# firechecking/CleanTransformer

Measured on AMD Instinct MI355X. Metric: SFT tokens/sec/step Bloom-560M bf16, higher is better.
Workload: dtype bf16

## Files before the change

### cleantransformer_amd/_lib.py

```python
from __future__ import annotations

import ctypes as C
import os

import torch

from ._build import LIB_PATH as _DEFAULT_LIB_PATH

LIB_PATH = os.environ.get("CTMI_LIB_PATH") or _DEFAULT_LIB_PATH

F32, BF16, F16 = 0, 1, 2
OPT_LEGACY_GRID = 4
OPT_SHADOW_F16 = 2
EPI_NONE, EPI_GELU, EPI_DGELU, EPI_RELU, EPI_DRELU, EPI_GELUG, EPI_MUL = 0, 1, 2, 3, 4, 5, 6
MT_MAX = 24
PROF_CLASSES = ("gemm_fwd", "gemm_dgrad", "gemm_wgrad", "lm_head", "attn_fwd", "attn_bwd", "layernorm", "loss", "optimizer", "reduce", "other")
ABI_VERSION = 16

vp, i64, i32, f32 = C.c_void_p, C.c_int64, C.c_int, C.c_float


class CtmiError(RuntimeError):
    pass


class AttnDesc(C.Structure):
    _fields_ = [(n, i64) for n in ("B", "nh", "Sq", "Sk", "hd",
                                   "q_bs", "q_hs", "q_rs", "k_bs", "k_hs", "k_rs",
                                   "v_bs", "v_hs", "v_rs", "o_bs", "o_hs", "o_rs",
                                   "am_b", "am_h", "am_q", "am_k")] + [("scale", f32), ("causal", i32), ("future_fill", f32), ("dropout_seed", C.c_uint32), ("dropout_p", f32), ("reserved_", i32)]


# ... 17 lines not shown


class BloomBlockGrads(C.Structure):
    _fields_ = [("dout", vp), ("dx", vp)] + [("d" + n, vp) for n in BLK_PARAMS] + \
               [("ws", vp), ("ws_bytes", i64), ("splitk_ws", vp), ("splitk_ws_bytes", i64), ("side_stream", vp),
                ("side_splitk_ws", vp), ("side_splitk_ws_bytes", i64), ("defer_join", i32)]


PROTOTYPES = {
    "ctmi_abi_version": (i32, []),
    "ctmi_last_error": (C.c_char_p, []),
    "ctmi_layernorm_fwd": (i32, [vp, vp, vp, vp, vp, vp, i64, i64, f32, i32, vp]),
    "ctmi_layernorm_bwd_ws": (i64, [i64, i64]),
    "ctmi_layernorm_bwd": (i32, [vp, vp, vp, vp, vp, vp, vp, vp, vp, i32, vp, i64, i64, i32, vp]),
    "ctmi_gemm": (i32, [vp, i64, i32, vp, i64, i32, vp, i64, i64, i64, i64, f32, i32, vp, vp, i32, vp, vp, i32, i32, vp, i64, vp]),
    "ctmi_set_launch_policy": (i32, [i32, i32]),
    "ctmi_get_launch_policy": (i32, [C.POINTER(i32), C.POINTER(i32)]),
    "ctmi_colsum": (i32, [vp, i64, vp, i32, vp, i64, i64, i32, vp]),
    "ctmi_colsum_ws": (i64, [i64, i64]),
    "ctmi_attn_fwd": (i32, [vp, vp, vp, vp, vp, vp, vp, vp, vp, vp, vp, C.POINTER(AttnDesc), i32, vp]),
    "ctmi_attn_bwd": (i32, [vp, vp, vp, vp, vp, vp, vp, vp, vp, vp, vp, vp, vp, vp, vp, vp, C.POINTER(AttnDesc), i32, vp]),
    "ctmi_attn_set_path": (i32, [i32]),
    "ctmi_mask_prep": (i32, [vp, vp, vp, vp, i64, i64, vp]),
    "ctmi_embed_fwd": (i32, [vp, vp, vp, i64, i64, i64, i32, vp, vp]),
    "ctmi_embed_bwd": (i32, [vp, vp, vp, i64, i64, i64, i32, f32, vp]),
    "ctmi_ce_fwd": (i32, [vp, i64, vp, vp, vp, vp, i64, i64, i64, i64, i64, i32, i64, i32, vp]),
    "ctmi_ce_bwd": (i32, [vp, i64, vp, vp, vp, vp, vp, i64, i64, i64, i64, i64, i64, i32, vp]),
    "ctmi_ce_fwd_bwd": (i32, [vp, i64, vp, vp, vp, vp, vp, i64, i64, i64, i64, i64, i64, i32, i64, f32, vp, i32, vp]),
    "ctmi_scale_if": (i32, [vp, i64, i64, i64, vp, f32, vp, i32, vp]),
    "ctmi_scale_if_passes": (i64, []),
# ... 13 lines not shown
    "ctmi_ddp_all_gather": (C.c_int, [C.c_void_p, C.c_void_p, C.c_void_p, C.c_int64, C.c_void_p]),
    "ctmi_ddp_broadcast": (C.c_int, [C.c_void_p, C.c_void_p, C.c_int64, C.c_int, C.c_void_p]),
    "ctmi_ddp_wait": (C.c_int, [C.c_void_p, C.c_void_p]),
    "ctmi_dropout_hash": (C.c_uint32, [C.c_uint32]),
    "ctmi_dropout_keep_hash": (C.c_uint32, [C.c_uint32, C.c_uint32]),
    "ctmi_dropout_threshold": (C.c_uint32, [f32]),
    "ctmi_dropout": (i32, [vp, vp, vp, i64, f32, C.c_uint32, i32, vp]),
    "ctmi_adamw_step": (i32, [C.POINTER(vp), C.POINTER(vp), C.POINTER(vp), C.POINTER(vp), C.POINTER(vp), C.POINTER(i64),
                              i32, f32, f32, f32, f32, f32, i32, i32, i32, f32, vp]),
    "ctmi_adamw_set_hyper": (i32, [vp, f32, f32, f32, f32, f32, i32, i32, i32, f32, vp]),
    "ctmi_adamw_step_dev": (i32, [C.POINTER(vp), C.POINTER(vp), C.POINTER(vp), C.POINTER(vp), C.POINTER(vp), C.POINTER(i64), i32, vp, vp]),
    "ctmi_sgd_step": (i32, [C.POINTER(vp), C.POINTER(vp), C.POINTER(vp), C.POINTER(vp), C.POINTER(i64),
                            i32, f32, f32, f32, f32, i32, vp]),
    "ctmi_cast": (i32, [vp, i32, vp, i32, i64, vp]),
    "ctmi_transpose_cast": (i32, [vp, vp, i32, i64, i64, vp]),
    "ctmi_sumsq": (i32, [vp, i64, vp, i32, vp]),
    "ctmi_scale": (i32, [vp, i64, f32, vp, vp]),
    "ctmi_scale_copy": (i32, [vp, vp, i64, f32, vp]),
    "ctmi_amp_unscale": (i32, [C.POINTER(vp), C.POINTER(i64), i32, vp, vp]),
    "ctmi_amp_update": (i32, [vp, f32, f32, i32, vp]),
    "ctmi_argmax": (i32, [vp, i64, vp, i64, i64, i32, vp]),
    "ctmi_row_lse": (i32, [vp, i64, vp, i64, i64, i32, vp]),
    "ctmi_group_topk": (i32, [vp, i64, vp, vp, f32, vp, vp, i64, i32, i64, i32, i32, vp]),
    "ctmi_scores_filter": (i32, [vp, i64, f32, vp, i64, f32, vp, i64, i64, i64, vp]),
    "ctmi_lora_project": (i32, [vp, i64, vp, i64, i32, vp, i64, i64, i64, i64, f32, i32, vp]),
    "ctmi_lora_expand_add": (i32, [vp, i64, vp, i64, i32, vp, i64, i64, i64, i64, i32, vp]),
    "ctmi_lora_wgrad_ws": (i64, [i64, i64, i64]),
    "ctmi_lora_wgrad": (i32, [vp, i64, vp, i64, vp, i64, i64, i64, i64, f32, vp, i64, i32, vp]),
    "ctmi_probe": (i32, [i32, vp, vp, vp]),
    "ctmi_clock_probe": (i32, [i32, vp, vp]),
# ... 42 lines not shown
```

### cleantransformer_amd/csrc/elementwise.hip

```cpp
#include "common.h"
#include "reduce_jobs.h"
#include "prof.h"
#include <hip/amd_detail/amd_hip_unsafe_atomics.h>

#ifndef CTMI_LN_BWD_PREFETCH
#define CTMI_LN_BWD_PREFETCH 1
#endif

static thread_local char g_err[512] = "";
void ctmi_set_error(const char* fmt, ...) {
    va_list ap; va_start(ap, fmt); vsnprintf(g_err, sizeof(g_err), fmt, ap); va_end(ap);
}
extern "C" const char* ctmi_last_error(void) { return g_err; }
static thread_local bool g_attr_err = false;
void ctmi_dyn_lds(const void* kern, size_t lds_bytes) {
    const hipError_t e = hipFuncSetAttribute(kern, hipFuncAttributeMaxDynamicSharedMemorySize, (int)lds_bytes);
    if (e != hipSuccess) {
        (void)hipGetLastError();
        ctmi_set_error("hipFuncSetAttribute(MaxDynamicSharedMemorySize = %zu bytes) refused: %s", lds_bytes, hipGetErrorString(e));
        g_attr_err = true;
    }
}
bool ctmi_take_attr_error() { const bool r = g_attr_err; g_attr_err = false; return r; }
extern "C" int ctmi_abi_version(void) { return CTMI_ABI_VERSION; }
// ... 1551 lines not shown
        if (c < C && r < R) dst[c * R + r] = Cvt<TD>::from_f(tile[tx][i]);
    }
}
extern "C" int ctmi_transpose_cast(const float* src, void* dst, int dst_dtype, int64_t rows, int64_t cols, void* stream) {
    ProfScope prof__(CTMI_PROF_OTHER, as_stream(stream));
    CTMI_REQUIRE(src && dst && rows > 0 && cols > 0, "transpose_cast: bad args");
    const dim3 grid((unsigned)cdiv64(cols, 64), (unsigned)cdiv64(rows, 64));
    if (dst_dtype == CTMI_F32) hipLaunchKernelGGL((transpose_cast_k<float>), grid, dim3(256), 0, as_stream(stream), src, (float*)dst, rows, cols);
    else if (dst_dtype == CTMI_BF16) hipLaunchKernelGGL((transpose_cast_k<bf16_t>), grid, dim3(256), 0, as_stream(stream), src, (bf16_t*)dst, rows, cols);
    else if (dst_dtype == CTMI_F16) hipLaunchKernelGGL((transpose_cast_k<f16_t>), grid, dim3(256), 0, as_stream(stream), src, (f16_t*)dst, rows, cols);
    else { ctmi_set_error("transpose_cast: unsupported dtype %d", dst_dtype); return CTMI_ERR_UNSUPPORTED; }
    CTMI_CHECK_LAUNCH("transpose_cast");
    return CTMI_OK;
}

__global__ __launch_bounds__(256) void sumsq_k(const float* __restrict__ x, int64_t n, double* __restrict__ out) {
    double s = 0.0;
    for (int64_t i = (int64_t)blockIdx.x * 256 + threadIdx.x; i < n; i += (int64_t)gridDim.x * 256) { const double v = x[i]; s += v * v; }
    for (int o = 32; o > 0; o >>= 1) s += __shfl_xor(s, o, 64);
    __shared__ double sm[4];
    if ((threadIdx.x & 63) == 0) sm[threadIdx.x >> 6] = s;
    __syncthreads();
    if (threadIdx.x == 0) atomicAdd(out, sm[0] + sm[1] + sm[2] + sm[3]);
}
extern "C" int ctmi_sumsq(const float* x, int64_t n, double* out, int accumulate, void* stream) {
    ProfScope prof__(CTMI_PROF_OTHER, as_stream(stream));
    CTMI_REQUIRE(x && out && n >= 0, "sumsq: bad args");
    hipStream_t st = as_stream(stream);
    if (!accumulate) { if (hipMemsetAsync(out, 0, sizeof(double), st) != hipSuccess) { ctmi_set_error("sumsq: memset failed"); return CTMI_ERR_LAUNCH; } }
    if (n == 0) return CTMI_OK;
// ... 203 lines not shown
```

### cleantransformer_amd/csrc/gemm.hip

```cpp
#include "common.h"
#include "reduce_jobs.h"
#include <type_traits>
#include "mma.h"
#include "prof.h"
#include <atomic>
#ifndef CTMI_GEMM_PART
#define CTMI_GEMM_PART (-1)
#endif
#ifndef CTMI_GELU_AUX_WT
#define CTMI_GELU_AUX_WT 0
#endif
#ifndef CTMI_SIDE_PRE8
#define CTMI_SIDE_PRE8 1
#endif
#define CTMI_GEMM_HAS(p) (CTMI_GEMM_PART == -1 || CTMI_GEMM_PART == (p))

constexpr bool glds_k2(bool pp, int wm) { return pp && wm == 4; }
constexpr int glds_ring(bool pp, int wm, bool xlane = false) { return !pp ? 3 : (glds_k2(pp, wm) ? 6 : 4); }
constexpr int glds_patch_bytes(bool pp, int wm, bool xlane = false) { return (pp && !xlane && wm != 4) ? 4 * 8192 : 0; }


template <typename T> struct Tile;
template <> struct Tile<bf16_t> { static constexpr int BM = 128, BN = 128, BK = 64, PADK = 8, PADR = 8; };
template <> struct Tile<f16_t>  { static constexpr int BM = 128, BN = 128, BK = 64, PADK = 8, PADR = 8; };
// ... 103 lines not shown
    return tile[(r16 + (lane & 15)) * PITCH + kofs];
}
template <> __device__ __forceinline__ float OpTile<float, true, 128>::frag(const float* __restrict__ tile, int r16, int lane, int kofs) {
    return tile[kofs * PITCH + r16 + (lane & 15)];
}

struct GemmArgs {
    const void* A; const void* B; void* C;
    int64_t lda, ldb, ldc, M, N, K;
    float alpha; int beta;
    const float* bias; const void* residual; const void* aux_in; void* aux_out;
    int tiles_m, tiles_n, vec_c, vec8;
    int nt_c;
    int splits; int64_t k_per_split; float* slabs;
    int splitk_ok; float* ws; int64_t ws_bytes;
};

constexpr int WG_MAXP = 4;
struct GroupProb { const void* A; const void* B; float* C; float* cs; float* part; float* cspart; int64_t lda, ldb, ldc, M, N, csn; };
struct GroupedArgs : GemmArgs { GroupProb p[WG_MAXP]; const int4* items; int nitems; };
constexpr int WG_PART = 16, WG_COLSUM = 32, WG_HALF1 = 64, WG_COLSUMB = 128;
template <bool GRP, int WM, bool BSUM = false> struct GrpRegs { };
template <int WM> struct GrpRegs<true, WM, false> { f32x4 accs; bool cs_on; };
template <int WM> struct GrpRegs<true, WM, true> { f32x4 accs; bool cs_on; f32x4 accb[4]; bool csb_on; };
#define WG_ONES8 (std::is_same<T, f16_t>::value ? short8{0x3C00, 0x3C00, 0x3C00, 0x3C00, 0x3C00, 0x3C00, 0x3C00, 0x3C00} \
                                                : short8{0x3F80, 0x3F80, 0x3F80, 0x3F80, 0x3F80, 0x3F80, 0x3F80, 0x3F80})

typedef uint32_t u32x4 __attribute__((ext_vector_type(4)));
template <typename TO> __device__ __forceinline__ void store4(TO* p, const float* v);
template <> __device__ __forceinline__ void store4<float>(float* p, const float* v) { *reinterpret_cast<float4*>(p) = make_float4(v[0], v[1], v[2], v[3]); }
// ... 226 lines not shown

template <typename TO, bool AK, bool BKM, int EPI, int WM, int WGN, bool PP, bool RES, bool XLANE, bool GRP, typename GA, typename TE = bf16_t, bool BSUM = false>
__device__ __forceinline__ void glds_body(const GA g) {
    using T = TE;
    static_assert(!GRP || (PP && WM == 4 && WGN == 4 && AK && BKM && EPI == CTMI_EPI_NONE && sizeof(TO) == 4), "grouped launches: weight gradients on the 128x256 ping-pong tile");
    constexpr int NW = 2 * WGN;
    constexpr int BM = WM * 32, BN = WGN * 64, BK = 32, NST = glds_ring(PP, WM, XLANE);
    using TA = GTile<AK, BM>;
    using TB = GTile<BKM, BN>;
    constexpr int STAGE = TA::BYTES + TB::BYTES;
    constexpr int AOFF = 0, BOFF = NST * TA::BYTES;
    constexpr int PA = TA::NINSTR / NW, PB = TB::NINSTR / NW;
    constexpr int LOADS = PA + PB;
    static_assert(PP ? (LOADS == 3 || LOADS == 4) : (LOADS == 4 || LOADS == 6), "vmcnt immediates below assume these DMA piece counts");
    constexpr bool K2 = glds_k2(PP, WM);
    constexpr int FILL = K2 ? NST - 2 : NST - 1;
    constexpr int LAND = K2 ? 2 : 1;
    extern __shared__ __attribute__((aligned(16))) unsigned char smem_raw[];

    const int tiles_m = (int)((g.M + BM - 1) / BM);
    const int tiles_n = (int)((g.N + BN - 1) / BN);
    const int ntile = tiles_m * tiles_n;
    int nwork_;
    if constexpr (GRP) nwork_ = g.nitems; else nwork_ = ntile * g.splits;
    const int nwork = nwork_;
    const int bid = blockIdx.x, G = gridDim.x;
    constexpr int GM = (WM == 8) ? ((AK && BKM) ? 1 : 4) : 8;
    auto decode = [&](int w, int64_t& m0, int64_t& n0, int& split) {
        const int xcd = w & 7, q = nwork >> 3, r8 = nwork & 7;
        const int vid_all = (xcd < r8 ? xcd * (q + 1) : r8 * (q + 1) + (xcd - r8) * q) + (w >> 3);
// ... 114 lines not shown
                float* d = Cl + (int64_t)arow(i) * ldc + 32 * jp;
                st_wt16(d, f32x4{a0, a1, a2, a3});
                st_wt16(d + 4, f32x4{b0, b1, b2, b3});
            }
        if (gs.cs_on) {
            if ((lane >> 4) == 0) {
                float* d = (part ? P.cspart + (half1 ? P.csn : 0) : P.cs) + mw + arow(0) + lane;
                *d = gs.accs[0];
            }
        }
        if constexpr (BSUM) {
            if (gs.csb_on && (lane & 15) == 0) {
                float* d = (part ? P.cspart + (half1 ? P.csn : 0) : P.cs) + nw + (lane >> 4) * 4;
#pragma unroll
                for (int j = 0; j < 4; ++j) *reinterpret_cast<f32x4*>(d + j * 16) = gs.accb[j];
            }
        }
        return;
    }
    if (g.splits > 1) {
        float* S = g.slabs + (int64_t)split * g.M * g.N;
#pragma unroll
        for (int i = 0; i < WM; ++i) {
            const int64_t m = m0 + wr * (WM * 16) + i * 16 + (lane & 15);
            if (m >= g.M) continue;
#pragma unroll
            for (int j = 0; j < 4; ++j) {
                const int64_t n = n0 + wc * 64 + j * 16 + (lane >> 4) * 4;
                if (n >= g.N) continue;
                float v[4] = {acc[i][j][0], acc[i][j][1], acc[i][j][2], acc[i][j][3]};
// ... 401 lines not shown
                    const unsigned char* bs = smem_raw + BOFF + rd * TB::BYTES;
                    short8 af[WM], bf[4];
#pragma unroll
                    for (int j = 0; j < 4; ++j) bf[j] = TB::frag(bs, wc * 64 + j * 16, lane);
#pragma unroll
                    for (int i = 0; i < WM; ++i) af[i] = TA::frag(as, wr * (WM * 16) + arow(i), lane);
                    issue_stage(wrb);
                    wait_stages(FILL - LAND);
                    asm volatile("s_waitcnt lgkmcnt(0)" ::: "memory");
                    __builtin_amdgcn_sched_barrier(0);
                    __builtin_amdgcn_s_barrier();
                    __builtin_amdgcn_sched_barrier(0);
#pragma unroll
                    for (int i = 0; i < WM; ++i)
#pragma unroll
                        for (int j = 0; j < 4; ++j) acc[i][j] = Mma<T>::mma(bf[j], af[i], acc[i][j]);
                    if constexpr (GRP) {
                        if (gs.cs_on) gs.accs = Mma<T>::mma(WG_ONES8, af[0], gs.accs);
                        if constexpr (BSUM) {
                            if (gs.csb_on) {
#pragma unroll
                                for (int j = 0; j < 4; ++j) gs.accb[j] = Mma<T>::mma(bf[j], WG_ONES8, gs.accb[j]);
                            }
                        }
                    }
                    __builtin_amdgcn_sched_barrier(0);
                    __builtin_amdgcn_s_barrier();
                    __builtin_amdgcn_sched_barrier(0);
                    if constexpr ((NST & (NST - 1)) == 0) { rd = (rd + 1) & (NST - 1); wrb = (wrb + 1) & (NST - 1); }
                    else { rd = rd == NST - 1 ? 0 : rd + 1; wrb = wrb == NST - 1 ? 0 : wrb + 1; }
                }
// ... 11 lines not shown
            for (int j = 0; j < 4; ++j) bf[j] = TB::frag(bs, wc * 64 + j * 16, lane);
#pragma unroll
            for (int i = 0; i < WM; ++i) af[i] = TA::frag(as, wr * (WM * 16) + arow(i), lane);
            if (more) {
                issue_stage(wrb);
                stage_issued(); ++inflight; wrb = wrb == NST - 1 ? 0 : wrb + 1;
            }
            wait_stages(inflight - 1 - LAND);
            asm volatile("s_waitcnt lgkmcnt(0)" ::: "memory");
            __builtin_amdgcn_sched_barrier(0);
            __builtin_amdgcn_s_barrier();
            __builtin_amdgcn_sched_barrier(0);
#pragma unroll
            for (int i = 0; i < WM; ++i)
#pragma unroll
                for (int j = 0; j < 4; ++j) acc[i][j] = Mma<T>::mma(bf[j], af[i], acc[i][j]);
            if constexpr (GRP) {
                if (gs.cs_on) gs.accs = Mma<T>::mma(WG_ONES8, af[0], gs.accs);
                if constexpr (BSUM) {
                    if (gs.csb_on) {
#pragma unroll
                        for (int j = 0; j < 4; ++j) gs.accb[j] = Mma<T>::mma(bf[j], WG_ONES8, gs.accb[j]);
                    }
                }
            }
            __builtin_amdgcn_sched_barrier(0);
            __builtin_amdgcn_s_barrier();
            __builtin_amdgcn_sched_barrier(0);
            rd = rd == NST - 1 ? 0 : rd + 1;
            --inflight;
            if (++tc < ntc) continue;
// ... 315 lines not shown
    if (g.splits > 1) {
        const int64_t total = g.M * g.N;
        const unsigned rg = (unsigned)std::min<int64_t>(cdiv64(total, 256), 4096);
        hipLaunchKernelGGL((splitk_reduce<TO>), dim3(rg), dim3(256), 0, st, g.slabs, reinterpret_cast<TO*>(g.C), g.ldc, g.M, g.N, g.splits, g.alpha, g.beta);
        CTMI_CHECK_LAUNCH("gemm_splitk_reduce");
    }
    return CTMI_OK;
}

int ctmi_gemm_bf16_nt(GemmArgs& g, int epi, bool fast, hipStream_t st);
int ctmi_gemm_bf16_nn(GemmArgs& g, int epi, bool fast, hipStream_t st);
int ctmi_gemm_bf16_tn(GemmArgs& g, int epi, bool fast, hipStream_t st);
int ctmi_gemm_f16_nt(GemmArgs& g, int epi, bool fast, hipStream_t st);
int ctmi_gemm_f16_nn(GemmArgs& g, int epi, bool fast, hipStream_t st);
int ctmi_gemm_f16_tn(GemmArgs& g, int epi, bool fast, hipStream_t st);
static int gemm_unsupported(int ak, int bk, int epi, int out_f32) {
    ctmi_set_error("gemm: unsupported combination a_kmajor=%d b_kmajor=%d epilogue=%d out_f32=%d", ak, bk, epi, out_f32);
    return CTMI_ERR_UNSUPPORTED;
}

#if CTMI_GEMM_HAS(1)
int ctmi_gemm_bf16_nt(GemmArgs& g, int epi, bool fast, hipStream_t st) {
    if (epi == CTMI_EPI_NONE) return gemm_launch<bf16_t, bf16_t, false, false, CTMI_EPI_NONE>(g, fast, st);
    if (epi == CTMI_EPI_GELU) return gemm_launch<bf16_t, bf16_t, false, false, CTMI_EPI_GELU>(g, fast, st);
    if (epi == CTMI_EPI_GELUG) return gemm_launch<bf16_t, bf16_t, false, false, CTMI_EPI_GELUG>(g, fast, st);
    if (epi == CTMI_EPI_RELU) return gemm_launch<bf16_t, bf16_t, false, false, CTMI_EPI_RELU>(g, fast, st);
    if (epi == CTMI_EPI_DGELU) return gemm_launch<bf16_t, bf16_t, false, false, CTMI_EPI_DGELU>(g, fast, st);
    return gemm_unsupported(0, 0, epi, 0);
}
#endif
#if CTMI_GEMM_HAS(2)
int ctmi_gemm_bf16_nn(GemmArgs& g, int epi, bool fast, hipStream_t st) {
    if (epi == CTMI_EPI_NONE) return gemm_launch<bf16_t, bf16_t, false, true, CTMI_EPI_NONE>(g, fast, st);
    if (epi == CTMI_EPI_DGELU) return gemm_launch<bf16_t, bf16_t, false, true, CTMI_EPI_DGELU>(g, fast, st);
    if (epi == CTMI_EPI_MUL) return gemm_launch<bf16_t, bf16_t, false, true, CTMI_EPI_MUL>(g, fast, st);
    if (epi == CTMI_EPI_DRELU) return gemm_launch<bf16_t, bf16_t, false, true, CTMI_EPI_DRELU>(g, fast, st);
    if (epi == CTMI_EPI_GELU) return gemm_launch<bf16_t, bf16_t, false, true, CTMI_EPI_GELU>(g, fast, st);
    return gemm_unsupported(0, 1, epi, 0);
}
#endif
#if CTMI_GEMM_HAS(3)
int ctmi_gemm_bf16_tn(GemmArgs& g, int epi, bool fast, hipStream_t st) {
    if (epi == CTMI_EPI_NONE) return gemm_launch<bf16_t, float, true, true, CTMI_EPI_NONE>(g, fast, st);
    return gemm_unsupported(1, 1, epi, 1);
}

#include <map>
#include <mutex>
#include <vector>
namespace {
struct WgShape { int64_t M[WG_MAXP], N[WG_MAXP]; int cs[WG_MAXP]; int n; int64_t ksteps; int slots; int split;
    bool operator<(const WgShape& o) const {
        if (n != o.n) return n < o.n;
        if (ksteps != o.ksteps) return ksteps < o.ksteps;
        if (slots != o.slots) return slots < o.slots;
        if (split != o.split) return split < o.split;
        for (int i = 0; i < n; ++i) { if (M[i] != o.M[i]) return M[i] < o.M[i]; if (N[i] != o.N[i]) return N[i] < o.N[i]; if (cs[i] != o.cs[i]) return cs[i] < o.cs[i]; }
        return false;
    }
};
// ... 192 lines not shown
int ctmi_gemm_f16_nn(GemmArgs& g, int epi, bool fast, hipStream_t st) {
    using T = f16_t;
    if (epi == CTMI_EPI_NONE) return gemm_launch<T, T, false, true, CTMI_EPI_NONE>(g, fast, st);
    if (epi == CTMI_EPI_DGELU) return gemm_launch<T, T, false, true, CTMI_EPI_DGELU>(g, fast, st);
    if (epi == CTMI_EPI_MUL) return gemm_launch<T, T, false, true, CTMI_EPI_MUL>(g, fast, st);
    if (epi == CTMI_EPI_DRELU) return gemm_launch<T, T, false, true, CTMI_EPI_DRELU>(g, fast, st);
    if (epi == CTMI_EPI_GELU) return gemm_launch<T, T, false, true, CTMI_EPI_GELU>(g, fast, st);
    return gemm_unsupported(0, 1, epi, 0);
}
#endif
#if CTMI_GEMM_HAS(6)
int ctmi_gemm_f16_tn(GemmArgs& g, int epi, bool fast, hipStream_t st) {
    if (epi == CTMI_EPI_NONE) return gemm_launch<f16_t, float, true, true, CTMI_EPI_NONE>(g, fast, st);
    return gemm_unsupported(1, 1, epi, 1);
}
#endif

#if CTMI_GEMM_HAS(0)
static int gemm_dispatch_bf16(GemmArgs& g, int ak, int bk, int epi, int out_f32, bool fast, hipStream_t st) {
    if (!ak && !bk && !out_f32) return ctmi_gemm_bf16_nt(g, epi, fast, st);
    if (!ak && bk && !out_f32) return ctmi_gemm_bf16_nn(g, epi, fast, st);
    if (ak && bk && out_f32) return ctmi_gemm_bf16_tn(g, epi, fast, st);
    return gemm_unsupported(ak, bk, epi, out_f32);
}

static int gemm_dispatch_f16(GemmArgs& g, int ak, int bk, int epi, int out_f32, bool fast, hipStream_t st) {
    if (!ak && !bk && !out_f32) return ctmi_gemm_f16_nt(g, epi, fast, st);
    if (!ak && bk && !out_f32) return ctmi_gemm_f16_nn(g, epi, fast, st);
    if (ak && bk && out_f32) return ctmi_gemm_f16_tn(g, epi, fast, st);
    return gemm_unsupported(ak, bk, epi, out_f32);
}

static int gemm_dispatch_f32(GemmArgs& g, int ak, int bk, int epi, bool fast, hipStream_t st) {
    using T = float;
    if (!ak && !bk) {
        if (epi == CTMI_EPI_NONE) return gemm_launch<T, float, false, false, CTMI_EPI_NONE>(g, fast, st);
        if (epi == CTMI_EPI_GELU) return gemm_launch<T, float, false, false, CTMI_EPI_GELU>(g, fast, st);
        if (epi == CTMI_EPI_GELUG) return gemm_launch<T, float, false, false, CTMI_EPI_GELUG>(g, fast, st);
        if (epi == CTMI_EPI_RELU) return gemm_launch<T, float, false, false, CTMI_EPI_RELU>(g, fast, st);
        if (epi == CTMI_EPI_DGELU) return gemm_launch<T, float, false, false, CTMI_EPI_DGELU>(g, fast, st);
    }
    if (!ak && bk) {
        if (epi == CTMI_EPI_NONE) return gemm_launch<T, float, false, true, CTMI_EPI_NONE>(g, fast, st);
        if (epi == CTMI_EPI_DGELU) return gemm_launch<T, float, false, true, CTMI_EPI_DGELU>(g, fast, st);
        if (epi == CTMI_EPI_MUL) return gemm_launch<T, float, false, true, CTMI_EPI_MUL>(g, fast, st);
        if (epi == CTMI_EPI_DRELU) return gemm_launch<T, float, false, true, CTMI_EPI_DRELU>(g, fast, st);
        if (epi == CTMI_EPI_GELU) return gemm_launch<T, float, false, true, CTMI_EPI_GELU>(g, fast, st);
    }
    if (ak && bk && epi == CTMI_EPI_NONE) return gemm_launch<T, float, true, true, CTMI_EPI_NONE>(g, fast, st);
    return gemm_unsupported(ak, bk, epi, 1);
}

extern "C" int ctmi_gemm(const void* A, int64_t lda, int a_kmajor, const void* B, int64_t ldb, int b_kmajor,
                         void* C, int64_t ldc, int64_t M, int64_t N, int64_t K,
                         float alpha, int beta, const float* bias, const void* residual, int epilogue,
                         const void* aux_in, void* aux_out, int out_f32, int dtype,
                         void* workspace, int64_t workspace_bytes, void* stream) {
    CTMI_REQUIRE(A && B && C, "gemm: null operand");
    CTMI_REQUIRE(M > 0 && N > 0 && K > 0, "gemm: bad shape M=%lld N=%lld K=%lld", (long long)M, (long long)N, (long long)K);
    CTMI_REQUIRE(lda >= (a_kmajor ? M : K) && ldb >= (b_kmajor ? N : K) && ldc >= N, "gemm: leading dimension too small");
    CTMI_REQUIRE((epilogue != CTMI_EPI_GELU && epilogue != CTMI_EPI_GELUG) || aux_out, "gemm: GELU epilogues need aux_out");
    CTMI_REQUIRE((epilogue != CTMI_EPI_DGELU && epilogue != CTMI_EPI_DRELU && epilogue != CTMI_EPI_MUL) || aux_in, "gemm: dGELU/dReLU/MUL epilogues need aux_in");
    CTMI_REQUIRE(dtype == CTMI_F32 || dtype == CTMI_BF16 || dtype == CTMI_F16, "gemm: unsupported dtype %d", dtype);
    ProfScope prof__((M >= 65536 || N >= 65536 || K >= 65536) ? CTMI_PROF_LM_HEAD
                     : (a_kmajor && b_kmajor ? CTMI_PROF_GEMM_WGRAD : ((!a_kmajor && b_kmajor) ? CTMI_PROF_GEMM_DGRAD : CTMI_PROF_GEMM_FWD)), as_stream(stream));
    const int es = dtype == CTMI_F32 ? 4 : 2;
    const int vec = 16 / es;
    const int bkt = dtype == CTMI_F32 ? Tile<float>::BK : Tile<bf16_t>::BK;
    GemmArgs g;
    g.A = A; g.B = B; g.C = C; g.lda = lda; g.ldb = ldb; g.ldc = ldc; g.M = M; g.N = N; g.K = K;
    g.alpha = alpha; g.beta = beta; g.bias = bias; g.residual = residual; g.aux_in = aux_in; g.aux_out = aux_out;
    g.tiles_m = (int)cdiv64(M, 128); g.tiles_n = (int)cdiv64(N, 128);
    const int64_t ntile = (int64_t)g.tiles_m * g.tiles_n;
    CTMI_REQUIRE(ntile < (1LL << 27), "gemm: too many tiles");
    const bool vec_a = (lda % vec == 0) && ((((uintptr_t)A) & 15) == 0) && ((a_kmajor ? M : K) % vec == 0);
    const bool vec_b = (ldb % vec == 0) && ((((uintptr_t)B) & 15) == 0) && ((b_kmajor ? N : K) % vec == 0);
    const bool fast = vec_a && vec_b;
    auto al = [](const void* p, int bytes) { return p == nullptr || ((((uintptr_t)p) & (bytes - 1)) == 0); };
    const int cbytes = (out_f32 || dtype == CTMI_F32) ? 16 : 8;
    g.vec_c = (ldc % 4 == 0) && al(C, cbytes) && al(residual, 4 * es) && al(aux_in, 4 * es) && al(aux_out, 4 * es) && al(bias, 16);
    static int nt_on = -1;
    if (nt_on < 0) { const char* e = getenv("CTMI_GEMM_NT"); nt_on = e ? atoi(e) : 1; }
    g.nt_c = nt_on && (M * N * (int64_t)((out_f32 || dtype == CTMI_F32) ? 4 : 2) > (1LL << 30)) ? 1 : 0;
    g.vec8 = g.vec_c && (ldc % 8 == 0) && al(C, 16) && al(residual, 16) && al(aux_in, 16) && al(aux_out, 16);
    g.splits = 1; g.k_per_split = K; g.slabs = nullptr;
    g.splitk_ok = (workspace != nullptr && epilogue == CTMI_EPI_NONE && bias == nullptr && residual == nullptr) ? 1 : 0;
    g.ws = reinterpret_cast<float*>(workspace); g.ws_bytes = workspace_bytes;
    if (workspace != nullptr && epilogue == CTMI_EPI_NONE && bias == nullptr && residual == nullptr && ntile < 384 && K >= 8 * bkt) {
        int64_t want = std::min<int64_t>(8, cdiv64(512, ntile));
        want = std::min<int64_t>(want, K / (4 * bkt));
        want = std::min<int64_t>(want, workspace_bytes / (int64_t)(M * N * sizeof(float)));
        if (want > 1) {
            const int64_t kps = cdiv64(cdiv64(K, want), bkt) * bkt;
            g.splits = (int)cdiv64(K, kps); g.k_per_split = kps; g.slabs = reinterpret_cast<float*>(workspace);
            if (g.splits <= 1) { g.splits = 1; g.k_per_split = K; g.slabs = nullptr; }
        }
    }
    if (dtype == CTMI_F32) return gemm_dispatch_f32(g, a_kmajor, b_kmajor, epilogue, fast, as_stream(stream));
    if (dtype == CTMI_F16) return gemm_dispatch_f16(g, a_kmajor, b_kmajor, epilogue, out_f32, fast, as_stream(stream));
    return gemm_dispatch_bf16(g, a_kmajor, b_kmajor, epilogue, out_f32, fast, as_stream(stream));
}
#endif

#if CTMI_GEMM_PART == 9
#ifndef CTMI_ONE_KERNEL
#define CTMI_ONE_KERNEL bf16_t, false, true, 0, 4, 4, true, false, false
#endif
template __global__ void gemm_glds_kernel<CTMI_ONE_KERNEL>(GemmArgs);
#endif
```

### cleantransformer_amd/models/modeling_bloom.py

```python
from __future__ import annotations

import math
import os as _os
from typing import Optional

import torch

from .. import _lib, ops, rng
from ..generation.generation_util import GenerationMixin
from ..transformer import LayerNorm

Tensor = torch.Tensor


class BloomConfig():

    def __init__(
            self,
            vocab_size=250880,
            hidden_size=64,
            n_layer=2,
            num_attention_heads=8,
            layer_norm_epsilon=1e-5,
            initializer_range=0.02,
# ... 297 lines not shown
        h2, weight = ctx.saved_tensors
        B, S, H = ctx.shape
        V = weight.shape[0]
        d2 = dlogits.reshape(B * S, V)
        wc = ops.compute_weight(weight, h2.dtype)
        tie = ctx.tie
        tied = tie is not None and tie.embed_wants
        sync = getattr(weight, "_ct_tied_sync", None) if tied else None
        pre = sync.prescale(weight) if sync is not None else None
        Vp = ops.ZERO_PADDED.pop(d2.data_ptr(), (None, None))[0] if d2.is_cuda else None
        want_dw = ctx.needs_input_grad[1]
        wpad = getattr(weight, "_ct_shadow_pad", None)
        if Vp is not None and d2.stride() == (Vp, 1) and wpad is not None and wpad.shape[0] == Vp and wpad.dtype == h2.dtype:
            dp = d2.as_strided((B * S, Vp), (Vp, 1))
            dh = ops.linear_dgrad(dp, wpad)
            dw = ops.linear_wgrad(dp, h2, alpha=1.0 if pre is None else pre)[:V] if want_dw else None
        else:
            d2 = ops._c(d2)
            rows = sync.chunk_rows(V, H) if pre is not None else V
            if rows < V:
                dw = torch.empty((V, H), dtype=torch.float32, device=d2.device)
                sync.announce(tie.n_tokens, d2.device)
                for c0 in range(0, V, rows):
                    c1 = min(V, c0 + rows)
                    ops.gemm(d2[:, c0:], V, True, h2, H, True, c1 - c0, H, B * S, out=dw[c0:c1], out_f32=True, alpha=pre)
                    sync.begin(dw[c0:c1])
                tie.pending, tie.early = dw, sync
                dh = ops.linear_dgrad(d2, wc)
                return dh.view(B, S, H), None, None
            dh = ops.linear_dgrad(d2, wc)
            dw = ops.linear_wgrad(d2, h2, alpha=1.0 if pre is None else pre) if want_dw else None
        if tied:
            tie.pending = dw
            if pre is not None:
                sync.announce(tie.n_tokens, dw.device)
                sync.begin(dw)
                tie.early = sync
            dw = None
        return dh.view(B, S, H), dw, None


_FUSED_CE = _os.environ.get("CTMI_FUSED_CE", "1") != "0"


class ShiftedCrossEntropyFn(torch.autograd.Function):

# ... 209 lines not shown
```

### cleantransformer_amd/ops.py

```python
from __future__ import annotations

import contextlib
import os
import ctypes as C
import math
import threading
from typing import Optional, Tuple

import torch

from . import _lib
from ._lib import AttnDesc, BF16, F16, F32, check

Tensor = torch.Tensor


def _p(t: Optional[Tensor]):
    return None if t is None else C.c_void_p(t.data_ptr())


def _stream():
    return C.c_void_p(torch.cuda.current_stream().cuda_stream)


# ... 143 lines not shown
def linear_fwd(x2d: Tensor, w: Tensor, bias: Optional[Tensor] = None, residual: Optional[Tensor] = None,
               epilogue: int = _lib.EPI_NONE, aux_out: Optional[Tensor] = None, tag: Optional[str] = None,
               out: Optional[Tensor] = None) -> Tensor:
    T, K = x2d.shape
    N = w.shape[0]
    return gemm(x2d, K, False, w, K, False, T, N, K, bias=bias, residual=residual, epilogue=epilogue, aux_out=aux_out, tag=tag, out=out)


def linear_dgrad(dy: Tensor, w: Tensor, epilogue: int = _lib.EPI_NONE, aux_in: Optional[Tensor] = None,
                 residual: Optional[Tensor] = None) -> Tensor:
    T, Nout = dy.shape
    Kin = w.shape[1]
    return gemm(dy, Nout, False, w, Kin, True, T, Kin, Nout, epilogue=epilogue, aux_in=aux_in, residual=residual)


def linear_wgrad(dy: Tensor, x2d: Tensor, out: Optional[Tensor] = None, accumulate: bool = False, alpha: float = 1.0) -> Tensor:
    T, Nout = dy.shape
    Kin = x2d.shape[1]
    return gemm(dy, Nout, True, x2d, Kin, True, Nout, Kin, T, out=out, out_f32=True, beta=int(accumulate), alpha=alpha)


def wgrad_grouped(problems, in_out: bool = False):
    lib = _lib.load()
    arr = (_lib.WgradProblem * len(problems))()
    outs = []
    T = problems[0][0].shape[0]
    for i, (dy, x, want_db) in enumerate(problems):
        _need_cuda(dy, x)
        assert dy.is_contiguous() and x.is_contiguous() and dy.shape[0] == T and x.shape[0] == T
        n_out, n_in = dy.shape[1], x.shape[1]
        dw = torch.empty((n_in, n_out) if in_out else (n_out, n_in), dtype=torch.float32, device=dy.device)
        db = torch.empty(n_out, dtype=torch.float32, device=dy.device) if want_db else None
        arr[i].dy, arr[i].x, arr[i].dw, arr[i].db = dy.data_ptr(), x.data_ptr(), dw.data_ptr(), (None if db is None else db.data_ptr())
        arr[i].n_out, arr[i].n_in, arr[i].in_out = n_out, n_in, int(in_out)
# ... 871 lines not shown
```

### include/ctmi355.h

```cpp
#ifndef CTMI355_H
#define CTMI355_H

#include <stdint.h>

#ifdef __cplusplus
extern "C" {
#endif

#define CTMI_ABI_VERSION 16

enum ctmi_dtype { CTMI_F32 = 0, CTMI_BF16 = 1, CTMI_F16 = 2 };
enum ctmi_status { CTMI_OK = 0, CTMI_ERR_ARG = -1, CTMI_ERR_LAUNCH = -2, CTMI_ERR_UNSUPPORTED = -3 };

int ctmi_abi_version(void);
const char* ctmi_last_error(void);

int ctmi_layernorm_fwd(const void* x, const float* w, const float* b, void* y, float* mean, float* rstd,
                       int64_t rows, int64_t cols, float eps, int dtype, void* stream);
int64_t ctmi_layernorm_bwd_ws(int64_t rows, int64_t cols);
int ctmi_layernorm_bwd(const void* dy, const void* x, const float* w, const float* mean, const float* rstd,
                       const void* dres, void* dx, float* dw, float* db, int accumulate, float* ws,
                       int64_t rows, int64_t cols, int dtype, void* stream);

enum ctmi_epilogue { CTMI_EPI_NONE = 0, CTMI_EPI_GELU = 1, CTMI_EPI_DGELU = 2, CTMI_EPI_RELU = 3, CTMI_EPI_DRELU = 4,
                     CTMI_EPI_GELUG = 5, CTMI_EPI_MUL = 6 };
int ctmi_gemm(const void* A, int64_t lda, int a_kmajor, const void* B, int64_t ldb, int b_kmajor,
              void* C, int64_t ldc, int64_t M, int64_t N, int64_t K,
              float alpha, int beta, const float* bias, const void* residual, int epilogue,
              const void* aux_in, void* aux_out, int out_f32, int dtype,
              void* workspace, int64_t workspace_bytes, void* stream);

typedef struct ctmi_wgrad_problem {
    const void* dy; const void* x;
    float* dw; float* db;
    int64_t n_out, n_in;
    int in_out; int pad_;
} ctmi_wgrad_problem;
int ctmi_wgrad_grouped(const ctmi_wgrad_problem* problems , int count, int64_t T, int dtype,
                       void* workspace , int64_t workspace_bytes, void* stream);

int ctmi_set_launch_policy(int shared, int reserve_cus);
int ctmi_get_launch_policy(int* shared , int* reserve_cus );

enum ctmi_prof_class {
    CTMI_PROF_GEMM_FWD = 0,
// ... 84 lines not shown
                    int decoupled, int mutate_grad, float grad_scale, void* stream);
int ctmi_adamw_set_hyper(void* hyper_dev , float lr, float beta1, float beta2, float eps, float weight_decay,
                         int step, int decoupled, int mutate_grad, float grad_scale, void* stream);
int ctmi_adamw_step_dev(float* const* p , float* const* g , float* const* m , float* const* v ,
                        void* const* shadow , const int64_t* n , int count,
                        const void* hyper_dev , void* stream);
int ctmi_sgd_step(float* const* p, float* const* g, float* const* buf ,
                  void* const* shadow, const int64_t* n, int count, float lr, float momentum, float dampening,
                  float weight_decay, int first_step, void* stream);

int ctmi_amp_unscale(float* const* g , const int64_t* n , int count, float* state , void* stream);
int ctmi_amp_update(float* state , float growth, float backoff, int interval, void* stream);

int ctmi_cast(const void* src, int src_dtype, void* dst, int dst_dtype, int64_t n, void* stream);
int ctmi_transpose_cast(const float* src, void* dst, int dst_dtype, int64_t rows, int64_t cols, void* stream);
int ctmi_sumsq(const float* x, int64_t n, double* out, int accumulate, void* stream);
int ctmi_scale(float* x, int64_t n, float s, const float* s_dev , void* stream);
int ctmi_scale_copy(const float* src, float* dst, int64_t n, float s, void* stream);
int ctmi_argmax(const void* x, int64_t ld, int64_t* out, int64_t rows, int64_t cols, int dtype, void* stream);

int ctmi_row_lse(const void* x, int64_t ld, float* stats , int64_t rows, int64_t cols, int dtype, void* stream);
int ctmi_group_topk(const void* x, int64_t ld, const float* stats, const float* add, float add_mul, float* out_val ,
                    int64_t* out_idx , int64_t groups, int group, int64_t cols, int k, int dtype, void* stream);
int ctmi_scores_filter(const float* x, int64_t ld, float divisor, const float* thr, int64_t thr_stride, float fill, float* out,
                       int64_t ldo, int64_t rows, int64_t cols, void* stream);

#define CTMI_REDUCE_MAX_JOBS 16
typedef struct ctmi_reduce_job {
    const float* src; float* dst; int64_t n; int64_t part_stride; int32_t nparts; int32_t accumulate; float alpha; int32_t pad_;
} ctmi_reduce_job;
// ... 55 lines not shown
```

Measured before the change: 230,800.

## Compute LM-head weight gradient via transposed activations and transposed-output NN GEMM

Adds a 16-bit tiled transpose kernel and a new GEMM variant that computes the LM-head weight gradient in NN form over pre-transposed hidden states, storing the fp32 result transposed by swapping MMA operands. The old path used the TN (both k-major) wgrad kernel for the large vocab x hidden product. The intent is to use the faster NN ping-pong tile path for this large GEMM, paying for it with one extra transpose of the hidden activations and an extra buffer. A fallback to the original GEMM remains when shapes or alignment do not qualify.

Result: no change. 231,500 (median of 6 runs) (+0.3%).

```diff
diff --git a/cleantransformer_amd/_lib.py b/cleantransformer_amd/_lib.py
--- a/cleantransformer_amd/_lib.py
+++ b/cleantransformer_amd/_lib.py
@@ -15,7 +15,7 @@
 EPI_NONE, EPI_GELU, EPI_DGELU, EPI_RELU, EPI_DRELU, EPI_GELUG, EPI_MUL = 0, 1, 2, 3, 4, 5, 6
 MT_MAX = 24
 PROF_CLASSES = ("gemm_fwd", "gemm_dgrad", "gemm_wgrad", "lm_head", "attn_fwd", "attn_bwd", "layernorm", "loss", "optimizer", "reduce", "other")
-ABI_VERSION = 16
+ABI_VERSION = 17
 
 vp, i64, i32, f32 = C.c_void_p, C.c_int64, C.c_int, C.c_float
 
@@ -63,6 +63,7 @@
     "ctmi_layernorm_bwd_ws": (i64, [i64, i64]),
     "ctmi_layernorm_bwd": (i32, [vp, vp, vp, vp, vp, vp, vp, vp, vp, i32, vp, i64, i64, i32, vp]),
     "ctmi_gemm": (i32, [vp, i64, i32, vp, i64, i32, vp, i64, i64, i64, i64, f32, i32, vp, vp, i32, vp, vp, i32, i32, vp, i64, vp]),
+    "ctmi_lmhead_wgrad": (i32, [vp, i64, vp, i64, vp, i64, i64, i64, i64, f32, i32, vp]),
     "ctmi_set_launch_policy": (i32, [i32, i32]),
     "ctmi_get_launch_policy": (i32, [C.POINTER(i32), C.POINTER(i32)]),
     "ctmi_colsum": (i32, [vp, i64, vp, i32, vp, i64, i64, i32, vp]),
@@ -106,6 +107,7 @@
                             i32, f32, f32, f32, f32, i32, vp]),
     "ctmi_cast": (i32, [vp, i32, vp, i32, i64, vp]),
     "ctmi_transpose_cast": (i32, [vp, vp, i32, i64, i64, vp]),
+    "ctmi_transpose16": (i32, [vp, i64, vp, i64, i64, i64, vp]),
     "ctmi_sumsq": (i32, [vp, i64, vp, i32, vp]),
     "ctmi_scale": (i32, [vp, i64, f32, vp, vp]),
     "ctmi_scale_copy": (i32, [vp, vp, i64, f32, vp]),
diff --git a/cleantransformer_amd/csrc/elementwise.hip b/cleantransformer_amd/csrc/elementwise.hip
--- a/cleantransformer_amd/csrc/elementwise.hip
+++ b/cleantransformer_amd/csrc/elementwise.hip
@@ -1589,6 +1589,48 @@
     return CTMI_OK;
 }
 
+__global__ __launch_bounds__(256) void transpose16_k(const uint16_t* __restrict__ src, int64_t ld_src, uint16_t* __restrict__ dst, int64_t ld_dst,
+                                                     int64_t R, int64_t C) {
+    __shared__ uint32_t tile[64 * 33];
+    const int t = threadIdx.x;
+    const int64_t r0 = (int64_t)blockIdx.y * 64, c0 = (int64_t)blockIdx.x * 64;
+#pragma unroll
+    for (int i = 0; i < 2; ++i) {
+        const int id = t + 256 * i, row = id >> 3, cc = id & 7;
+        const int64_t r = r0 + row, c = c0 + cc * 8;
+        if (r < R && c < C) {
+            const uint4 v = *reinterpret_cast<const uint4*>(src + r * ld_src + c);
+            uint32_t* d = tile + row * 33 + cc * 4;
+            d[0] = v.x; d[1] = v.y; d[2] = v.z; d[3] = v.w;
+        }
+    }
+    __syncthreads();
+    const int rc = t & 7, cp = t >> 3;
+    const int64_t r = r0 + rc * 8, c = c0 + cp * 2;
+    if (r < R && c < C) {
+        uint32_t w[8];
+#pragma unroll
+        for (int k = 0; k < 8; ++k) w[k] = tile[(rc * 8 + k) * 33 + cp];
+        uint4 lo, hi;
+        lo.x = (w[0] & 0xffffu) | (w[1] << 16); lo.y = (w[2] & 0xffffu) | (w[3] << 16); lo.z = (w[4] & 0xffffu) | (w[5] << 16); lo.w = (w[6] & 0xffffu) | (w[7] << 16);
+        hi.x = (w[0] >> 16) | (w[1] & 0xffff0000u); hi.y = (w[2] >> 16) | (w[3] & 0xffff0000u); hi.z = (w[4] >> 16) | (w[5] & 0xffff0000u); hi.w = (w[6] >> 16) | (w[7] & 0xffff0000u);
+        *reinterpret_cast<uint4*>(dst + c * ld_dst + r) = lo;
+        *reinterpret_cast<uint4*>(dst + (c + 1) * ld_dst + r) = hi;
+    }
+}
+extern "C" int ctmi_transpose16(const void* src, int64_t ld_src, void* dst, int64_t ld_dst, int64_t rows, int64_t cols, void* stream) {
+    ProfScope prof__(CTMI_PROF_OTHER, as_stream(stream));
+    CTMI_REQUIRE(src && dst && rows > 0 && cols > 0 && ld_src >= cols && ld_dst >= rows, "transpose16: bad args");
+    if ((rows | cols | ld_src | ld_dst) % 8 != 0 || !aligned16(src) || !aligned16(dst) || cdiv64(rows, 64) > 65535) {
+        ctmi_set_error("transpose16: rows, cols and both row pitches must be multiples of 8 and the pointers 16-byte aligned (rows <= 4193280)");
+        return CTMI_ERR_UNSUPPORTED;
+    }
+    const dim3 grid((unsigned)cdiv64(cols, 64), (unsigned)cdiv64(rows, 64));
+    hipLaunchKernelGGL(transpose16_k, grid, dim3(256), 0, as_stream(stream), (const uint16_t*)src, ld_src, (uint16_t*)dst, ld_dst, rows, cols);
+    CTMI_CHECK_LAUNCH("transpose16");
+    return CTMI_OK;
+}
+
 __global__ __launch_bounds__(256) void sumsq_k(const float* __restrict__ x, int64_t n, double* __restrict__ out) {
     double s = 0.0;
     for (int64_t i = (int64_t)blockIdx.x * 256 + threadIdx.x; i < n; i += (int64_t)gridDim.x * 256) { const double v = x[i]; s += v * v; }
diff --git a/cleantransformer_amd/csrc/gemm.hip b/cleantransformer_amd/csrc/gemm.hip
--- a/cleantransformer_amd/csrc/gemm.hip
+++ b/cleantransformer_amd/csrc/gemm.hip
@@ -141,6 +141,7 @@
     int nt_c;
     int splits; int64_t k_per_split; float* slabs;
     int splitk_ok; float* ws; int64_t ws_bytes;
+    int trans_c;
 };
 
 constexpr int WG_MAXP = 4;
@@ -397,6 +398,12 @@
     constexpr int LOADS = PA + PB;
     static_assert(PP ? (LOADS == 3 || LOADS == 4) : (LOADS == 4 || LOADS == 6), "vmcnt immediates below assume these DMA piece counts");
     constexpr bool K2 = glds_k2(PP, WM);
+    constexpr bool TRC = sizeof(TO) == 4 && !AK && BKM && !GRP;
+    static_assert(!TRC || (PP && WM == 8 && WGN == 4 && EPI == CTMI_EPI_NONE && !RES && !XLANE), "transposed fp32 output: the 256x256 ping-pong tile, plain epilogue");
+    auto mma_ab = [&](const short8& a, const short8& b, const f32x4& c) __attribute__((always_inline)) {
+        if constexpr (TRC) return Mma<T>::mma(a, b, c);
+        else return Mma<T>::mma(b, a, c);
+    };
     constexpr int FILL = K2 ? NST - 2 : NST - 1;
     constexpr int LAND = K2 ? 2 : 1;
     extern __shared__ __attribute__((aligned(16))) unsigned char smem_raw[];
@@ -541,6 +548,30 @@
                 float* d = (part ? P.cspart + (half1 ? P.csn : 0) : P.cs) + nw + (lane >> 4) * 4;
 #pragma unroll
                 for (int j = 0; j < 4; ++j) *reinterpret_cast<f32x4*>(d + j * 16) = gs.accb[j];
+            }
+        }
+        return;
+    }
+    if constexpr (TRC) {
+        float* Ct = reinterpret_cast<float*>(g.C);
+        const int64_t mw = m0 + wr * (WM * 16) + (lane >> 4) * 4, nw = n0 + wc * 64 + (lane & 15);
+        if ((m0 + BM <= g.M) && (n0 + BN <= g.N)) {
+            float* Cl = Ct + nw * g.ldc + mw;
+            const int64_t row16 = 16 * g.ldc;
+#pragma unroll
+            for (int j = 0; j < 4; ++j)
+#pragma unroll
+                for (int i = 0; i < WM; ++i) st_wt16(Cl + j * row16 + i * 16, acc[i][j] * g.alpha);
+        } else {
+#pragma unroll
+            for (int j = 0; j < 4; ++j) {
+                const int64_t n = nw + j * 16;
+                if (n >= g.N) continue;
+#pragma unroll
+                for (int i = 0; i < WM; ++i) {
+                    const int64_t m = mw + i * 16;
+                    if (m < g.M) st_wt16(Ct + n * g.ldc + m, acc[i][j] * g.alpha);
+                }
             }
         }
         return;
@@ -972,7 +1003,7 @@
 #pragma unroll
                     for (int i = 0; i < WM; ++i)
 #pragma unroll
-                        for (int j = 0; j < 4; ++j) acc[i][j] = Mma<T>::mma(bf[j], af[i], acc[i][j]);
+                        for (int j = 0; j < 4; ++j) acc[i][j] = mma_ab(af[i], bf[j], acc[i][j]);
                     if constexpr (GRP) {
                         if (gs.cs_on) gs.accs = Mma<T>::mma(WG_ONES8, af[0], gs.accs);
                         if constexpr (BSUM) {
@@ -1014,7 +1045,7 @@
 #pragma unroll
             for (int i = 0; i < WM; ++i)
 #pragma unroll
-                for (int j = 0; j < 4; ++j) acc[i][j] = Mma<T>::mma(bf[j], af[i], acc[i][j]);
+                for (int j = 0; j < 4; ++j) acc[i][j] = mma_ab(af[i], bf[j], acc[i][j]);
             if constexpr (GRP) {
                 if (gs.cs_on) gs.accs = Mma<T>::mma(WG_ONES8, af[0], gs.accs);
                 if constexpr (BSUM) {
@@ -1360,9 +1391,25 @@
 int ctmi_gemm_f16_nt(GemmArgs& g, int epi, bool fast, hipStream_t st);
 int ctmi_gemm_f16_nn(GemmArgs& g, int epi, bool fast, hipStream_t st);
 int ctmi_gemm_f16_tn(GemmArgs& g, int epi, bool fast, hipStream_t st);
+int ctmi_gemm_bf16_nn_tc(GemmArgs& g, int epi, bool fast, hipStream_t st);
+int ctmi_gemm_f16_nn_tc(GemmArgs& g, int epi, bool fast, hipStream_t st);
 static int gemm_unsupported(int ak, int bk, int epi, int out_f32) {
     ctmi_set_error("gemm: unsupported combination a_kmajor=%d b_kmajor=%d epilogue=%d out_f32=%d", ak, bk, epi, out_f32);
     return CTMI_ERR_UNSUPPORTED;
+}
+
+template <typename T>
+static int gemm_launch_nn_tc(GemmArgs& g, int epi, bool fast, hipStream_t st) {
+    const bool ok = g.trans_c && epi == CTMI_EPI_NONE && fast && glds_enabled() && g.K % 32 == 0 && g.M % 4 == 0 && g.vec_c && !g.beta &&
+                    g.bias == nullptr && g.residual == nullptr;
+    if (!ok) {
+        ctmi_set_error("gemm: the transposed-output form needs 16-bit operands, 16-byte aligned pointers, K %% 32 == 0, M %% 4 == 0, ldc %% 4 == 0 and a plain epilogue");
+        return CTMI_ERR_UNSUPPORTED;
+    }
+    g.splits = 1; g.k_per_split = g.K; g.slabs = nullptr;
+    glds_launch<T, float, false, true, CTMI_EPI_NONE, 8, 4, true>(g, st);
+    CTMI_CHECK_LAUNCH("gemm_glds_nn_tc");
+    return CTMI_OK;
 }
 
 #if CTMI_GEMM_HAS(1)
@@ -1390,6 +1437,7 @@
     if (epi == CTMI_EPI_NONE) return gemm_launch<bf16_t, float, true, true, CTMI_EPI_NONE>(g, fast, st);
     return gemm_unsupported(1, 1, epi, 1);
 }
+int ctmi_gemm_bf16_nn_tc(GemmArgs& g, int epi, bool fast, hipStream_t st) { return gemm_launch_nn_tc<bf16_t>(g, epi, fast, st); }
 
 #include <map>
 #include <mutex>
@@ -1612,6 +1660,7 @@
     if (epi == CTMI_EPI_NONE) return gemm_launch<f16_t, float, true, true, CTMI_EPI_NONE>(g, fast, st);
     return gemm_unsupported(1, 1, epi, 1);
 }
+int ctmi_gemm_f16_nn_tc(GemmArgs& g, int epi, bool fast, hipStream_t st) { return gemm_launch_nn_tc<f16_t>(g, epi, fast, st); }
 #endif
 
 #if CTMI_GEMM_HAS(0)
@@ -1619,6 +1668,7 @@
     if (!ak && !bk && !out_f32) return ctmi_gemm_bf16_nt(g, epi, fast, st);
     if (!ak && bk && !out_f32) return ctmi_gemm_bf16_nn(g, epi, fast, st);
     if (ak && bk && out_f32) return ctmi_gemm_bf16_tn(g, epi, fast, st);
+    if (!ak && bk && out_f32 && g.trans_c) return ctmi_gemm_bf16_nn_tc(g, epi, fast, st);
     return gemm_unsupported(ak, bk, epi, out_f32);
 }
 
@@ -1626,6 +1676,7 @@
     if (!ak && !bk && !out_f32) return ctmi_gemm_f16_nt(g, epi, fast, st);
     if (!ak && bk && !out_f32) return ctmi_gemm_f16_nn(g, epi, fast, st);
     if (ak && bk && out_f32) return ctmi_gemm_f16_tn(g, epi, fast, st);
+    if (!ak && bk && out_f32 && g.trans_c) return ctmi_gemm_f16_nn_tc(g, epi, fast, st);
     return gemm_unsupported(ak, bk, epi, out_f32);
 }
 
@@ -1649,14 +1700,14 @@
     return gemm_unsupported(ak, bk, epi, 1);
 }
 
-extern "C" int ctmi_gemm(const void* A, int64_t lda, int a_kmajor, const void* B, int64_t ldb, int b_kmajor,
-                         void* C, int64_t ldc, int64_t M, int64_t N, int64_t K,
-                         float alpha, int beta, const float* bias, const void* residual, int epilogue,
-                         const void* aux_in, void* aux_out, int out_f32, int dtype,
-                         void* workspace, int64_t workspace_bytes, void* stream) {
+static int gemm_entry(const void* A, int64_t lda, int a_kmajor, const void* B, int64_t ldb, int b_kmajor,
+                      void* C, int64_t ldc, int64_t M, int64_t N, int64_t K,
+                      float alpha, int beta, const float* bias, const void* residual, int epilogue,
+                      const void* aux_in, void* aux_out, int out_f32, int dtype,
+                      void* workspace, int64_t workspace_bytes, void* stream, int trans_c) {
     CTMI_REQUIRE(A && B && C, "gemm: null operand");
     CTMI_REQUIRE(M > 0 && N > 0 && K > 0, "gemm: bad shape M=%lld N=%lld K=%lld", (long long)M, (long long)N, (long long)K);
-    CTMI_REQUIRE(lda >= (a_kmajor ? M : K) && ldb >= (b_kmajor ? N : K) && ldc >= N, "gemm: leading dimension too small");
+    CTMI_REQUIRE(lda >= (a_kmajor ? M : K) && ldb >= (b_kmajor ? N : K) && ldc >= (trans_c ? M : N), "gemm: leading dimension too small");
     CTMI_REQUIRE((epilogue != CTMI_EPI_GELU && epilogue != CTMI_EPI_GELUG) || aux_out, "gemm: GELU epilogues need aux_out");
     CTMI_REQUIRE((epilogue != CTMI_EPI_DGELU && epilogue != CTMI_EPI_DRELU && epilogue != CTMI_EPI_MUL) || aux_in, "gemm: dGELU/dReLU/MUL epilogues need aux_in");
     CTMI_REQUIRE(dtype == CTMI_F32 || dtype == CTMI_BF16 || dtype == CTMI_F16, "gemm: unsupported dtype %d", dtype);
@@ -1668,6 +1719,7 @@
     GemmArgs g;
     g.A = A; g.B = B; g.C = C; g.lda = lda; g.ldb = ldb; g.ldc = ldc; g.M = M; g.N = N; g.K = K;
     g.alpha = alpha; g.beta = beta; g.bias = bias; g.residual = residual; g.aux_in = aux_in; g.aux_out = aux_out;
+    g.trans_c = trans_c;
     g.tiles_m = (int)cdiv64(M, 128); g.tiles_n = (int)cdiv64(N, 128);
     const int64_t ntile = (int64_t)g.tiles_m * g.tiles_n;
     CTMI_REQUIRE(ntile < (1LL << 27), "gemm: too many tiles");
@@ -1694,9 +1746,25 @@
             if (g.splits <= 1) { g.splits = 1; g.k_per_split = K; g.slabs = nullptr; }
         }
     }
+    if (trans_c && dtype == CTMI_F32) return gemm_unsupported(a_kmajor, b_kmajor, epilogue, 1);
     if (dtype == CTMI_F32) return gemm_dispatch_f32(g, a_kmajor, b_kmajor, epilogue, fast, as_stream(stream));
     if (dtype == CTMI_F16) return gemm_dispatch_f16(g, a_kmajor, b_kmajor, epilogue, out_f32, fast, as_stream(stream));
     return gemm_dispatch_bf16(g, a_kmajor, b_kmajor, epilogue, out_f32, fast, as_stream(stream));
+}
+
+extern "C" int ctmi_gemm(const void* A, int64_t lda, int a_kmajor, const void* B, int64_t ldb, int b_kmajor,
+                         void* C, int64_t ldc, int64_t M, int64_t N, int64_t K,
+                         float alpha, int beta, const float* bias, const void* residual, int epilogue,
+                         const void* aux_in, void* aux_out, int out_f32, int dtype,
+                         void* workspace, int64_t workspace_bytes, void* stream) {
+    return gemm_entry(A, lda, a_kmajor, B, ldb, b_kmajor, C, ldc, M, N, K, alpha, beta, bias, residual, epilogue, aux_in, aux_out, out_f32, dtype,
+                      workspace, workspace_bytes, stream, 0);
+}
+
+extern "C" int ctmi_lmhead_wgrad(const void* dy, int64_t lddy, const void* xt, int64_t ldxt, float* dw, int64_t lddw,
+                                 int64_t V, int64_t H, int64_t T, float alpha, int dtype, void* stream) {
+    return gemm_entry(xt, ldxt, 0, dy, lddy, 1, dw, lddw, H, V, T, alpha, 0, nullptr, nullptr, CTMI_EPI_NONE, nullptr, nullptr, 1, dtype,
+                      nullptr, 0, stream, 1);
 }
 #endif
 
diff --git a/cleantransformer_amd/models/modeling_bloom.py b/cleantransformer_amd/models/modeling_bloom.py
--- a/cleantransformer_amd/models/modeling_bloom.py
+++ b/cleantransformer_amd/models/modeling_bloom.py
@@ -335,22 +335,23 @@
         if Vp is not None and d2.stride() == (Vp, 1) and wpad is not None and wpad.shape[0] == Vp and wpad.dtype == h2.dtype:
             dp = d2.as_strided((B * S, Vp), (Vp, 1))
             dh = ops.linear_dgrad(dp, wpad)
-            dw = ops.linear_wgrad(dp, h2, alpha=1.0 if pre is None else pre)[:V] if want_dw else None
+            dw = ops.lmhead_wgrad(dp, h2, alpha=1.0 if pre is None else pre)[:V] if want_dw else None
         else:
             d2 = ops._c(d2)
             rows = sync.chunk_rows(V, H) if pre is not None else V
             if rows < V:
                 dw = torch.empty((V, H), dtype=torch.float32, device=d2.device)
                 sync.announce(tie.n_tokens, d2.device)
+                ht = ops.lmhead_xt(h2)
                 for c0 in range(0, V, rows):
                     c1 = min(V, c0 + rows)
-                    ops.gemm(d2[:, c0:], V, True, h2, H, True, c1 - c0, H, B * S, out=dw[c0:c1], out_f32=True, alpha=pre)
+                    ops.lmhead_wgrad(d2[:, c0:c1], h2, out=dw[c0:c1], alpha=pre, xt=ht)
                     sync.begin(dw[c0:c1])
                 tie.pending, tie.early = dw, sync
                 dh = ops.linear_dgrad(d2, wc)
                 return dh.view(B, S, H), None, None
             dh = ops.linear_dgrad(d2, wc)
-            dw = ops.linear_wgrad(d2, h2, alpha=1.0 if pre is None else pre) if want_dw else None
+            dw = ops.lmhead_wgrad(d2, h2, alpha=1.0 if pre is None else pre) if want_dw else None
         if tied:
             tie.pending = dw
             if pre is not None:
diff --git a/cleantransformer_amd/ops.py b/cleantransformer_amd/ops.py
--- a/cleantransformer_amd/ops.py
+++ b/cleantransformer_amd/ops.py
@@ -181,10 +181,58 @@
     return gemm(dy, Nout, False, w, Kin, True, T, Kin, Nout, epilogue=epilogue, aux_in=aux_in, residual=residual)
 
 
-def linear_wgrad(dy: Tensor, x2d: Tensor, out: Optional[Tensor] = None, accumulate: bool = False, alpha: float = 1.0) -> Tensor:
+def linear_wgrad(dy: Tensor, x2d: Tensor, out: Optional[Tensor] = None, accumulate: bool = False, alpha: float = 1.0,
+                 xt: Optional[Tensor] = None) -> Tensor:
     T, Nout = dy.shape
     Kin = x2d.shape[1]
-    return gemm(dy, Nout, True, x2d, Kin, True, Nout, Kin, T, out=out, out_f32=True, beta=int(accumulate), alpha=alpha)
+    lda = dy.stride(0) if (T > 1 and dy.stride(1) == 1) else Nout
+    if xt is not None and not accumulate and dy.is_cuda and dy.dtype in (torch.bfloat16, torch.float16) and dy.stride(1) == 1:
+        if out is None:
+            out = torch.empty((Nout, Kin), dtype=torch.float32, device=dy.device)
+        rc = _lib.load().ctmi_lmhead_wgrad(_p(dy), lda, _p(xt), xt.stride(0), _p(out), out.stride(0), Nout, Kin, T, float(alpha),
+                                           dt_code(dy.dtype), _stream())
+        if rc == 0:
+            return out
+        if rc != _UNSUPPORTED:
+            check(rc, "lmhead_wgrad")
+    return gemm(dy, lda, True, x2d, Kin, True, Nout, Kin, T, out=out, out_f32=True, beta=int(accumulate), alpha=alpha)
+
+
+_UNSUPPORTED = -3
+LMHEAD_WGRAD_DEFAULT_FORM = "nn"
+
+
+def lmhead_wgrad_form() -> str:
+    f = os.environ.get("CTMI_LMHEAD_WGRAD_FORM", "").lower()
+    return f if f in ("nn", "tn") else LMHEAD_WGRAD_DEFAULT_FORM
+
+
+def transpose16(x: Tensor, out: Optional[Tensor] = None) -> Optional[Tensor]:
+    _need_cuda(x)
+    if x.dim() != 2 or x.dtype not in (torch.bfloat16, torch.float16) or x.stride(1) != 1:
+        return None
+    R, Cc = x.shape
+    if out is None:
+        out = torch.empty((Cc, R), dtype=x.dtype, device=x.device)
+    rc = _lib.load().ctmi_transpose16(_p(x), x.stride(0), _p(out), out.stride(0), R, Cc, _stream())
+    if rc == _UNSUPPORTED:
+        return None
+    check(rc, "transpose16")
+    return out
+
+
+def lmhead_xt(x2d: Tensor) -> Optional[Tensor]:
+    if lmhead_wgrad_form() != "nn" or not x2d.is_cuda:
+        return None
+    return transpose16(x2d)
+
+
+def lmhead_wgrad(dy: Tensor, x: Tensor, out: Optional[Tensor] = None, alpha: float = 1.0, xt: Optional[Tensor] = None) -> Tensor:
+    if lmhead_wgrad_form() != "nn":
+        xt = None
+    elif xt is None:
+        xt = lmhead_xt(x)
+    return linear_wgrad(dy, x, out=out, alpha=alpha, xt=xt)
 
 
 def wgrad_grouped(problems, in_out: bool = False):
diff --git a/include/ctmi355.h b/include/ctmi355.h
--- a/include/ctmi355.h
+++ b/include/ctmi355.h
@@ -7,7 +7,7 @@
 extern "C" {
 #endif
 
-#define CTMI_ABI_VERSION 16
+#define CTMI_ABI_VERSION 17
 
 enum ctmi_dtype { CTMI_F32 = 0, CTMI_BF16 = 1, CTMI_F16 = 2 };
 enum ctmi_status { CTMI_OK = 0, CTMI_ERR_ARG = -1, CTMI_ERR_LAUNCH = -2, CTMI_ERR_UNSUPPORTED = -3 };
@@ -29,6 +29,9 @@
               float alpha, int beta, const float* bias, const void* residual, int epilogue,
               const void* aux_in, void* aux_out, int out_f32, int dtype,
               void* workspace, int64_t workspace_bytes, void* stream);
+
+int ctmi_lmhead_wgrad(const void* dy, int64_t lddy, const void* xt, int64_t ldxt, float* dw, int64_t lddw,
+                      int64_t V, int64_t H, int64_t T, float alpha, int dtype, void* stream);
 
 typedef struct ctmi_wgrad_problem {
     const void* dy; const void* x;
@@ -143,6 +146,7 @@
 
 int ctmi_cast(const void* src, int src_dtype, void* dst, int dst_dtype, int64_t n, void* stream);
 int ctmi_transpose_cast(const float* src, void* dst, int dst_dtype, int64_t rows, int64_t cols, void* stream);
+int ctmi_transpose16(const void* src, int64_t ld_src, void* dst, int64_t ld_dst, int64_t rows, int64_t cols, void* stream);
 int ctmi_sumsq(const float* x, int64_t n, double* out, int accumulate, void* stream);
 int ctmi_scale(float* x, int64_t n, float s, const float* s_dev , void* stream);
 int ctmi_scale_copy(const float* src, float* dst, int64_t n, float s, void* stream);
```
